# zhibaishouheilab/HealthiVert-GAN

Measured on AMD Instinct MI355X. Metric: sagittal slices/sec (train step, G+D) at 256x256 bs=16, higher is better.
Workload: dtype f16; 1 GPU; two-stage coarse+refine generator + 3x PatchGAN D train step, 256x256, per-GPU bs=16, norm=batch, vanilla GAN; global_batch=16, parallelism=dp1, launch=hipGraph replay (1 graphs/step), 4 streams

## Files before the change

healthivert-gan_amd/csrc/build.py:

```python
import json
import os
import re
import subprocess
import sys
from concurrent.futures import ThreadPoolExecutor

HERE = os.path.dirname(os.path.abspath(__file__))
PKG = os.path.dirname(HERE)
ROOT = os.path.dirname(PKG)
HIPCC = os.environ.get('HIPCC', '/opt/rocm/bin/hipcc')
SOURCES = ['conv_igemm.hip', 'conv_halo.hip', 'conv_halo2.hip', 'conv_lf.hip', 'conv_g4.hip', 'conv_thin.hip', 'conv_px.hip', 'conv_s2t.hip', 'wgrad_halo.hip', 'wgrad_tr.hip', 'conv_narrow.hip', 'conv_head.hip', 'prep.hip', 'norm.hip', 'pointwise.hip', 'attention.hip', 'attention_gram.hip', 'bgemm.hip', 'rhlv.hip', 'assemble.hip', 'infer_prep.hip', 'eval_metrics.hip', 'straighten.hip', 'gen_eval.hip', 'depedicle.hip', 'svm_grade.hip', 'restore.hip', 'spline.hip', 'edt.hip', 'ccl3d.hip', 'morph.hip', 'labelstats.hip', 'filter3d.hip', 'rankfilt.hip', 'resample.hip', 'texture.hip', 'warp.hip', 'similarity.hip', 'shape.hip']
FLAGS = os.environ.get('HV_EXTRA_FLAGS', '').split() + ['--offload-arch=gfx950', '-O3', '-std=c++17', '-fPIC', '-ffp-contract=off', '-Wno-unused-result', '-Wno-inline-asm', '-Rpass-analysis=kernel-resource-usage']
OUT = os.path.join(PKG, 'libhvgan.so')


def _newer(src, dst, deps):
    if not os.path.exists(dst):
        return True
    t = os.path.getmtime(dst)
    return any(os.path.getmtime(p) > t for p in [src] + deps)


def _resources(remarks):
    out, cur = {}, None
    for line in remarks.splitlines():
        m = re.search(r'remark: (?:\S+ )?Function Name: (\S+)', line) or re.search(r'Function Name: (\S+)', line)
        if m:
            cur = out.setdefault(m.group(1), {})
            continue
        if cur is None:
            continue
        for key, pat in (('vgprs', r' VGPRs: (\d+)'), ('agprs', r'AGPRs: (\d+)'), ('scratch', r'ScratchSize \[bytes/lane\]: (\d+)'),
                         ('occupancy', r'Occupancy \[waves/SIMD\]: (\d+)'), ('lds', r'LDS Size \[bytes/block\]: (\d+)')):
            m = re.search(pat, line)
            if m:
                cur[key] = int(m.group(1))
    return out


def build(force=False, verbose=True):
    objdir = os.path.join(HERE, 'build')
    os.makedirs(objdir, exist_ok=True)
    deps = [os.path.join(HERE, 'hv_common.h'), os.path.join(HERE, 'conv_halo.h'), os.path.join(HERE, 'spline_tap.h'), os.path.join(HERE, 'boundary_map.h'), os.path.join(HERE, 'resample_core.h'), os.path.join(ROOT, 'include', 'hvgan.h')]
    jobs = []
    for s in SOURCES:
        src, obj = os.path.join(HERE, s), os.path.join(objdir, s.replace('.hip', '.o'))
        if force or _newer(src, obj, deps):
            jobs.append((src, obj))

    def cc(job):
        src, obj = job
        cmd = [HIPCC] + FLAGS + ['-c', src, '-o', obj]
        if verbose:
            print(' '.join(cmd), flush=True)
        r = subprocess.run(cmd, capture_output=True, text=True)
        if r.returncode != 0:
            raise RuntimeError('hipcc failed for %s:\n%s' % (src, r.stderr[-4000:]))
        with open(obj.replace('.o', '.resources.json'), 'w') as f:
            json.dump(_resources(r.stderr), f, indent=0, sort_keys=True)
        return r.stderr

    with ThreadPoolExecutor(max_workers=4) as ex:
        list(ex.map(cc, jobs))
    objs = [os.path.join(objdir, s.replace('.hip', '.o')) for s in SOURCES]
# ... 13 lines not shown
```

healthivert-gan_amd/csrc/prep.hip:

```cpp
#include <stdlib.h>

#include "hv_common.h"

#define SN_EPS 1e-12f
#define PREP_THREADS 512
#define PREP_MAXK 4608
#define PREP_MAXCO 1024

__device__ __forceinline__ long long wsrc_index(const hv_wprep_layer& L, int co, int ci, int tap) {
    return L.transposed_src ? ((long long)ci * L.Cout + co) * L.taps + tap : ((long long)co * L.Cin + ci) * L.taps + tap;
}

__global__ __launch_bounds__(PREP_THREADS) void weight_prep_kernel(const hv_wprep_layer* __restrict__ layers) {
    const hv_wprep_layer L = layers[blockIdx.x];
    __shared__ float v_s[PREP_MAXK];
    __shared__ float u_s[PREP_MAXCO];
    __shared__ float red[20];
    const int tid = threadIdx.x, lane = tid & 63, wave = tid >> 6, nwave = PREP_THREADS / 64;
    const int K = L.Cin * L.taps;
    float sigma = 1.f;
    if (L.sn) {
        const float* W = L.w_orig;
        for (int i = tid; i < L.Cout; i += PREP_THREADS) u_s[i] = L.u[i];
        for (int i = tid; i < K; i += PREP_THREADS) v_s[i] = L.v[i];
// ... 651 lines not shown
__global__ void fill_kernel(float* p, long long n, float v) {
    long long i = (long long)blockIdx.x * blockDim.x + threadIdx.x;
    const long long st = (long long)gridDim.x * blockDim.x;
    for (; i < n; i += st) p[i] = v;
}
__global__ void axpy_kernel(float* y, const float* x, long long n, float a, int assign) {
    long long i = (long long)blockIdx.x * blockDim.x + threadIdx.x;
    const long long st = (long long)gridDim.x * blockDim.x;
    for (; i < n; i += st) y[i] = assign ? a * x[i] : y[i] + a * x[i];
}
static int ew_grid(long long n) { long long b = (n + 255) / 256; return (int)(b > 4096 ? 4096 : (b < 1 ? 1 : b)); }
extern "C" int hv_fill(float* p, long long n, float value, void* stream) {
    if (!p || n <= 0) return HV_ERR_ARG;
    hipLaunchKernelGGL(fill_kernel, dim3(ew_grid(n)), dim3(256), 0, (hipStream_t)stream, p, n, value);
    HV_LAUNCH_CHECK();
    return HV_OK;
}
extern "C" int hv_axpy(float* y, const float* x, long long n, float a, void* stream) {
    if (!y || !x || n <= 0) return HV_ERR_ARG;
    hipLaunchKernelGGL(axpy_kernel, dim3(ew_grid(n)), dim3(256), 0, (hipStream_t)stream, y, x, n, a, 0);
    HV_LAUNCH_CHECK();
    return HV_OK;
}
__global__ void affine_kernel(float* y, const float* x, long long n, float a, float b) {
    long long i = (long long)blockIdx.x * blockDim.x + threadIdx.x;
    const long long st = (long long)gridDim.x * blockDim.x;
    for (; i < n; i += st) y[i] = a * x[i] + b;
}
extern "C" int hv_affine(float* y, const float* x, long long n, float a, float b, void* stream) {
    if (!y || !x || n <= 0) return HV_ERR_ARG;
    hipLaunchKernelGGL(affine_kernel, dim3(ew_grid(n)), dim3(256), 0, (hipStream_t)stream, y, x, n, a, b);
    HV_LAUNCH_CHECK();
    return HV_OK;
}

__global__ void mul_kernel(float* y, const float* x, const float* z, long long n) {
    long long i = (long long)blockIdx.x * blockDim.x + threadIdx.x;
    const long long st = (long long)gridDim.x * blockDim.x;
    for (; i < n; i += st) y[i] = z ? (y[i] * x[i]) * z[i] : y[i] * x[i];
}
extern "C" int hv_mul(float* y, const float* x, long long n, void* stream) {
    if (!y || !x || n <= 0) return HV_ERR_ARG;
    hipLaunchKernelGGL(mul_kernel, dim3(ew_grid(n)), dim3(256), 0, (hipStream_t)stream, y, x, (const float*)nullptr, n);
    HV_LAUNCH_CHECK();
    return HV_OK;
}
extern "C" int hv_mul3(float* y, const float* x, const float* z, long long n, void* stream) {
    if (!y || !x || !z || n <= 0) return HV_ERR_ARG;
    hipLaunchKernelGGL(mul_kernel, dim3(ew_grid(n)), dim3(256), 0, (hipStream_t)stream, y, x, z, n);
    HV_LAUNCH_CHECK();
    return HV_OK;
}

extern "C" int hv_version(void) { return 106; }
extern "C" const char* hv_arch(void) { return "gfx950"; }
```

healthivert-gan_amd/engine.py:

```python
import contextlib
import ctypes
import os
import types

import torch

from . import lib as _lib
from . import ops
from .lib import ptr, stream
from .ops import Act, rup


def precision_note(precision):
    if precision in ('fp16', 'f16'):
        return 'fp16 MFMA operands / fp32 accumulate; activations and gradients stored as fp16 (image tensors, attention scores, weights, statistics fp32)'
    return 'fp32 MFMA (v_mfma_f32_16x16x4_f32), fp32 storage'


SN_MAX_K, SN_MAX_COUT = 4608, 1024


class ConvParams:

    def __init__(self, name, weight, bias, cin, cout, k, cin_fwd=None, cin_wg=None, u=None, v=None, transposed_src=False):
# ... 300 lines not shown

    def mark(self, a):
        acc = self.accumulates(a)
        self.written.add((id(a.t), a.coff, a.C))
        return acc


class WgradBlock:
    __slots__ = ('side', 'collecting', 'queue', 'later', 'pset')

    def __init__(self):
        self.side, self.collecting, self.queue, self.later, self.pset = None, False, [], [], None

    def open(self, pset, device):
        fork = not SERIAL and torch.cuda.current_stream().cuda_stream not in NO_FORK_STREAMS
        self.side = named_stream('generator-wgrad-block', device) if fork else None
        self.collecting, self.queue, self.later, self.pset = fork, [], [], pset

    def add(self, run):
        self.queue.append(run)

    def before_next_block(self, run):
        if self.collecting:
            self.later.append(run)
        else:
            run()

    def launch(self, keep_collecting=False):
        if self.side is None:
            return
        self.side.wait_stream(torch.cuda.current_stream())
        with torch.cuda.stream(self.side):
            for run in self.queue:
                run()
            self.pset.fold_chain().flush()
        self.queue, self.later, self.collecting = self.later, [], keep_collecting

    def join(self):
        assert not self.queue and not self.later, 'WgradBlock.join(): queued weight gradients were never launched'
        if self.side is not None:
            torch.cuda.current_stream().wait_stream(self.side)
        self.side, self.collecting = None, False


def _wgrad(node, p, xin, gfull, accumulate, prec, dbias=None, dbias_accumulate=False):
    chain = p.owner.fold_chain() if p.owner is not None else None
    if node.transposed:
        ops.conv2d_wgrad(gfull, xin, p.dw, node.k, node.s, node.pad, node.d, accumulate=accumulate, precision=prec, chain=chain)
    else:
        ops.conv2d_wgrad(xin, gfull, p.dw, node.k, node.s, node.pad, node.d, in_shift=node.shift, accumulate=accumulate, precision=prec,
                         dbias=dbias, dbias_accumulate=dbias_accumulate, chain=chain)


def conv_backward(node, book, prec, dbias_accumulate=False, wgrad_accumulate=False, wgrad=True, x_wg=None, premultiplied=False,
                  mul_x=None, dbias_done=False, bn=None):
    p = node.p
    assert bn is None or (node.need_dx and not node.transposed and node.pool_to is None and not node.shift), 'conv_backward: bn= needs the plain data-gradient branch'
    gy = book.twin(node.y)
    want_dbias = p.bias is not None and node.use_bias and wgrad and not dbias_done
    fuse_dbias = want_dbias and not node.transposed and p.coutP == p.cout
    if (node.act != 'none' and not premultiplied) or (want_dbias and not fuse_dbias):
        ops.act_backward(gy, node.y, 'none' if premultiplied else node.act, dbias=p.bias.grad if (want_dbias and not fuse_dbias) else None, dbias_accumulate=dbias_accumulate)
    gfull = Act(gy.t, p.coutP, gy.coff)
    if wgrad:
        xs = node.x if x_wg is None else x_wg
        xin = Act(xs.t, p.cin_wg, xs.coff)
        if book.wgrad_block.collecting:
            book.wgrad_block.add(lambda node=node, p=p, xin=xin, gfull=gfull, acc=wgrad_accumulate, db=p.bias.grad if fuse_dbias else None, dba=dbias_accumulate:
                                 _wgrad(node, p, xin, gfull, acc, prec, dbias=db, dbias_accumulate=dba))
        else:
            _wgrad(node, p, xin, gfull, wgrad_accumulate, prec, dbias=p.bias.grad if fuse_dbias else None, dbias_accumulate=dbias_accumulate)
    if not node.need_dx:
        return
    if node.transposed:
        form = 'src'
    elif node.pool_to is not None and node.pooled(book, prec, 'pool_to'):
        form = 'pool_to'
    elif node.shift:
        form = 'pool' if node.pooled(book, prec, 'pool', mul_x) else 'full'
    else:
        form = 'plain'
    if form == 'full':
        assert not mul_x
        full = node.full_scratch()
        node.dx_call(book, prec, 'full', full, False).launch()
        gx = node.dx_view(book, 'plain')
        ops.copy_channels(full, gx, mode=3, accumulate=book.mark(gx))
    else:
        dst = node.dx_view(book, form)
        node.dx_call(book, prec, form, dst, book.mark(dst), mul_x=mul_x, bn=bn).launch()


_branch_streams = {}


def branch_stream():
    if SERIAL:
        return None
    cur = torch.cuda.current_stream()
    if cur.cuda_stream in NO_FORK_STREAMS:
        return None
    key = cur.device.index
    st = _branch_streams.get(key)
    if st is None:
        st = _branch_streams[key] = named_stream('generator-branch', cur.device)
        NO_FORK_STREAMS.add(st.cuda_stream)
    return st


def chain_link(n, nxt, book, prec):
    if not (nxt is not None and n.need_dx and not n.transposed and nxt.act != 'none'
            and n.x.t is nxt.y.t and n.x.coff == nxt.y.coff and n.p.cin_fwd <= nxt.y.t.shape[-1] - nxt.y.coff):
        return False
    return not n.shift or n.pooled(book, prec, 'pool', nxt.act)


def conv_backward_chain(nodes, book, prec, premultiplied_first=False, stop_before=None):
# ... 168 lines not shown
```

healthivert-gan_amd/models/networks.py:

```python
import functools

import torch
import torch.nn as nn
from torch.nn import init
from torch.optim import lr_scheduler

from ._backend import engine as E
from ._backend import lib as _lib
from ._backend import ops
Act, rup = ops.Act, ops.rup


class Identity(nn.Module):
    def forward(self, x):
        return x


def get_norm_layer(norm_type='instance'):
    if norm_type == 'batch':
        return functools.partial(nn.BatchNorm2d, affine=True, track_running_stats=True)
    if norm_type == 'instance':
        return functools.partial(nn.InstanceNorm2d, affine=False, track_running_stats=False)
    if norm_type == 'none':
        return lambda x: Identity()
# ... 53 lines not shown
    raise NotImplementedError('Generator model name [%s] is not recognized' % netG)


def define_D(input_nc, ndf, netD, n_layers_D=3, norm='batch', init_type='normal', init_gain=0.02, gpu_ids=[]):
    norm_layer = get_norm_layer(norm_type=norm)
    if netD == 'basic':
        net = NLayerDiscriminator(input_nc, ndf, n_layers=3, norm_layer=norm_layer)
    elif netD == 'n_layers':
        net = NLayerDiscriminator(input_nc, ndf, n_layers_D, norm_layer=norm_layer)
    elif netD in ('pixel', 'seg'):
        raise NotImplementedError("define_D('%s'): not on the HealthiVert-GAN hot path" % netD)
    else:
        raise NotImplementedError('Discriminator model name [%s] is not recognized' % netD)
    return init_net(net, init_type, init_gain, gpu_ids)


class _GanLossFn(torch.autograd.Function):
    @staticmethod
    def forward(ctx, pred, target_is_real, mode):
        loss = torch.zeros((), device=pred.device)
        dz = torch.empty_like(pred)
        ops.gan_loss(pred.contiguous(), target_is_real, mode, loss=loss, dz=dz)
        ctx.save_for_backward(dz)
        return loss

    @staticmethod
    def backward(ctx, g):
        (dz,) = ctx.saved_tensors
        return dz * g, None, None


class GANLoss(nn.Module):
    def __init__(self, gan_mode, target_real_label=1.0, target_fake_label=0.0):
        super().__init__()
        self.register_buffer('real_label', torch.tensor(target_real_label))
        self.register_buffer('fake_label', torch.tensor(target_fake_label))
        self.gan_mode = gan_mode
        if gan_mode not in ('lsgan', 'vanilla', 'wgangp'):
            raise NotImplementedError('gan mode %s not implemented' % gan_mode)
        if target_real_label != 1.0 or target_fake_label != 0.0:
            raise NotImplementedError("GANLoss HIP path: labels 1.0 / 0.0")

    def get_target_tensor(self, prediction, target_is_real):
        return (self.real_label if target_is_real else self.fake_label).expand_as(prediction)

    def __call__(self, prediction, target_is_real):
        if self.gan_mode == 'wgangp':
            raise NotImplementedError("GANLoss('wgangp') is not on the HealthiVert-GAN hot path")
        _lib.require_gpu(prediction)
        return _GanLossFn.apply(prediction, bool(target_is_real), self.gan_mode)


CONV_BSTATS = True
HEAD_NORM = True


class _Stem:
    __slots__ = ('p', 'y', 'node')

    def __init__(self, p, y):
        self.p, self.y, self.node = p, y, None


class _Normed:
    __slots__ = ('p', 'node', 'z', 'y', 'stats', 'norm', 'bparts_used', 'head_fused', '_fstats', '_bsums', '_head_ok')

    def __init__(self, p, node, z, y, stats, norm):
        self.p, self.node, self.z, self.y, self.stats, self.norm = p, node, z, y, stats, norm
        self.bparts_used = 0
        self.head_fused = False
        self._fstats = None
        self._bsums = {}
        self._head_ok = {}

    def _partials(self, parts):
        return torch.zeros(max(1, parts) * self.p.cout * 2, dtype=torch.float32, device=self.z.t.device), parts

    def forward_stats(self, prec):
        if self._fstats is None:
            self._fstats = self._partials(int(self.node.stats_parts(prec)))
        return self._fstats if self._fstats[1] else (None, 0)

    def backward_sums(self, consumer, book, prec, mul_x, groups):
        if groups not in self._bsums:
            gx = consumer.dx_view(book, 'plain')
            call = consumer.dx_call(book, prec, 'plain', gx, book.accumulates(gx), mul_x=mul_x, bn=(self.z, self.stats, groups, None))
            self._bsums[groups] = self._partials(call.bstats_parts())
        return self._bsums[groups] if self._bsums[groups][1] else (None, 0)

    def head_call(self, head, prec, groups):
        nm = self.norm
        bn = isinstance(nm, nn.BatchNorm2d)
        xn = (self.stats, nm.weight if bn else None, nm.bias if bn else None, groups if bn else self.z.B, 'lrelu', self.y)
        call = head.node.forward_call(prec, xn=xn, x_raw=self.z)
        if groups not in self._head_ok:
            self._head_ok[groups] = call.supported()
        return call if self._head_ok[groups] else None


class _Logits:
    __slots__ = ('p', 'node', 'y', 'carrier')

    def __init__(self, p, node, y, carrier):
        self.p, self.node, self.y, self.carrier = p, node, y, carrier

    @property
# ... 162 lines not shown
        head = P.layers[-1]
        if head.loss_head_ready:
            want_db = param_grads and head.p.bias is not None and head.node.use_bias
            args = [a for rows, real, loss in ranges for a in (P.logits[rows], real, loss, Act(head.carrier.t[rows], 4, 0))]
            ops.gan_loss_pair(*args, mode=mode, loss_weight=loss_weight, grad_weight=grad_weight, dbias=head.p.bias.grad if want_db else None,
                              dbias_accumulate=accumulate)
            return None, True
        if dz is None:
            dz = torch.empty_like(P.logits)
        for rows, real, loss in ranges:
            ops.gan_loss(P.logits[rows], real, mode, loss=loss, loss_weight=loss_weight, dz=dz[rows], grad_weight=grad_weight)
        return dz, False

    def loss_backward(self, P, target_is_real, mode, loss, grad_weight, need_dx=False, param_grads=True, accumulate=False, loss_weight=1.0, dz=None,
                      backward=True):
        dz, ready = self._loss_seed(P, [(slice(None), target_is_real, loss)], mode, grad_weight, loss_weight, param_grads, accumulate, dz)
        if not backward:
            return None
        return self.run_backward(P, dz, need_dx=need_dx, param_grads=param_grads, accumulate=accumulate, logits_ready=ready)

    def loss_backward_halves(self, P, mode, loss_fake, loss_real, grad_weight, dz=None):
        B = P.B // 2
        dz, ready = self._loss_seed(P, [(slice(0, B), False, loss_fake), (slice(B, None), True, loss_real)], mode, grad_weight, dz=dz)
        return self.run_backward(P, dz, need_dx=False, param_grads=True, accumulate=False, logits_ready=ready)

    def run_backward(self, P, dlogits, need_dx=False, param_grads=True, accumulate=False, logits_ready=False):
        prec = ops.precision_id(self.precision)
        book = P.book
        book.reset()
        B = P.B
        stem, head = P.layers[0], P.layers[-1]
        if not logits_ready:
            ops.copy_channels(Act(dlogits.contiguous().view(B, head.y.H, head.y.W, 1)), head.carrier, mode=0)
        bn = self.norm_kind == 'batch'
        fuse0 = stem.node.act != 'none' and not P.layers[1].node.shift
        sums = (None, 0)
        for li in range(len(P.layers) - 1, 0, -1):
            ent, below = P.layers[li], P.layers[li - 1]
            node = ent.node
            prev_normed = li >= 2 and not node.shift
            if ent is not head:
                nm = ent.norm
                ent.bparts_used = sums[1]
                ops.norm_act_backward(book.twin(ent.y), ent.y, ent.z, book.twin(ent.z), self.norm_kind, P.training, ent.stats,
                                      gamma=nm.weight if bn else None, act='none', dgamma=nm.weight.grad if (bn and param_grads) else None,
                                      dbeta=nm.bias.grad if (bn and param_grads) else None, param_accumulate=accumulate,
                                      groups=P.groups, partials=sums[0], n_partials=sums[1])
            mul_x = stem.node.act if (li == 1 and fuse0) else ('lrelu' if prev_normed else None)
            sums = (None, 0)
            if prev_normed and mul_x and CONV_BSTATS and bn and P.training:
                sums = below.backward_sums(node, book, prec, mul_x, P.groups)
            E.conv_backward(node, book, prec, dbias_accumulate=accumulate, wgrad_accumulate=accumulate, wgrad=param_grads, dbias_done=bool(logits_ready and ent is head),
                            mul_x=mul_x, bn=(below.z, below.stats, P.groups, sums[0]) if sums[1] else None)
        if param_grads:
            ops.copy_channels(P.x_in, P.x4, mode=0)
        stem.node.need_dx = need_dx
        E.conv_backward(stem.node, book, prec, dbias_accumulate=accumulate, wgrad_accumulate=accumulate, wgrad=param_grads,
                        x_wg=P.x4 if param_grads else None, premultiplied=fuse0)
        return book.twin(P.x_in).t.view(B, 1, P.H, P.W) if need_dx else None

    def finish(self):
        for P in self._plans.values():
            P.book.join()
        self.paramset().finish_backward(accumulate=False)
        self.paramset().attach_grads()

    def forward(self, input):
        if torch.is_grad_enabled() and (input.requires_grad or any(p.requires_grad for p in self.parameters())):
            B, _, H, W = input.shape
            P = self.run_forward(input, slot=self._free_plan_slot(B, H, W, input.device))
            anchor = next((p for p in self.parameters() if p.requires_grad), None)
            return _DiscFn.apply(input, anchor, self, P, P.logits)
        return self.run_forward(input).logits.clone()


class _PlanToken:
    """Alive as long as the autograd node that owns a plan's activations is."""


def grads_are_fresh(net):
    ps = list(net.parameters())
    fresh = getattr(ps[0], '_hv_fresh', False) or ps[0].grad is None
    for p in ps:
        p._hv_fresh = False
    return fresh


class _DiscFn(torch.autograd.Function):
    @staticmethod
    def forward(ctx, x, anchor, net, plan, logits):
        import weakref
        ctx.net, ctx.plan, ctx.need_dx = net, plan, x.requires_grad
        ctx.token = _PlanToken()
        plan.pending = weakref.ref(ctx.token)
        return logits.clone()

    @staticmethod
    def backward(ctx, g):
        net, plan = ctx.net, ctx.plan
        if plan.pending is None or plan.pending() is not ctx.token:
            raise RuntimeError("NLayerDiscriminator: the activations of this forward pass were overwritten before its backward ran")
        pg = any(p.requires_grad for p in net.parameters())
        acc = pg and not grads_are_fresh(net)
        S = ops.grad_scale(net.precision)
        pset = net.paramset()
        if acc:
            ops.scale_inplace(pset.flat_grad, S / pset.grad_factor)
        if pg:
            pset.attach_grads()
        dx = net.run_backward(plan, g.contiguous() * S if S != 1.0 else g.contiguous(), need_dx=ctx.need_dx, param_grads=pg, accumulate=acc)
        if pg:
# ... 8 lines not shown
```

healthivert-gan_amd/ops.py:

```python
import ctypes
import os

import torch

from . import lib as _lib
from .lib import ACT, NORM, F16, F32, ptr, stream

_PRECISION = {'fp32': F32, 'f32': F32, 'fp16': F16, 'f16': F16}


_TIMER = None


def timer():
    return _TIMER


def set_timer(t):
    global _TIMER
    _TIMER = t


def default_precision():
    return _PRECISION[os.environ.get('HV_PRECISION', 'fp32').lower()]
# ... 240 lines not shown
            _lib.get().call('hv_wgrad_fold_now', ctypes.byref(f), stream())


FOLD_CHAIN = True


def conv2d_wgrad(x, g, dw, k, stride=1, pad=0, dil=1, in_shift=0, accumulate=False, precision=None, cin=None, cout=None, dbias=None,
                 dbias_accumulate=False, chain=None):
    L = _lib.get()
    d = L.hv_wgrad_desc()
    kh, kw = (k, k) if isinstance(k, int) else k
    d.x = ptr(x.t).value
    d.B, d.H, d.W, d.in_shift = x.B, x.H << in_shift, x.W << in_shift, in_shift
    d.x_ld, d.x_coff, d.Cin = x.ld, x.coff, (x.C if cin is None else cin)
    d.g = ptr(g.t).value
    d.Ho, d.Wo, d.g_ld, d.g_coff, d.Cout = g.H, g.W, g.ld, g.coff, (g.C if cout is None else cout)
    d.KH, d.KW, d.stride, d.pad, d.dil = kh, kw, stride, pad, dil
    d.dw = ptr(dw).value
    d.accumulate = int(accumulate)
    d.precision = precision_id(precision)
    d.dbias = None if dbias is None else ptr(dbias).value
    d.dbias_accumulate = int(dbias_accumulate)
    d.x_f16, d.g_f16 = x.f16, g.f16
    d.workspace, d.workspace_bytes = None, 0
    if chain is not None and not FOLD_CHAIN:
        chain = None
    need = L.size('hv_conv2d_wgrad_workspace_bytes', ctypes.byref(d))
    fold = None
    if chain is not None:
        assert torch.cuda.current_stream(x.t.device).cuda_stream == chain.stream, 'a FoldChain belongs to one stream'
        if chain.pending is not None:
            d.carry = ctypes.pointer(chain.pending)
        if need:
            b, _ = _ws(need, x.t.device, slot=('fold-chain', chain.slot))
            chain.slot ^= 1
            d.workspace, d.workspace_bytes = ptr(b).value, b.numel()
            fold = L.hv_wgrad_fold()
            d.pending = ctypes.pointer(fold)
    elif need:
        b, _ = _ws(need, x.t.device)
        d.workspace, d.workspace_bytes = ptr(b).value, b.numel()
    if _TIMER is not None:
        flops = 2.0 * g.B * g.H * g.W * d.Cout * kh * kw * d.Cin
        nbytes = (2 if x.f16 else 4) * x.B * x.H * x.W * d.Cin + (2 if g.f16 else 4) * g.B * g.H * g.W * d.Cout + 4 * d.Cout * kh * kw * d.Cin
        _TIMER.wrap(('wgrad', x.B, d.H, d.W, d.Cin, d.Cout, kh, stride, dil, 0), flops,
                    lambda: L.call('hv_conv2d_wgrad', ctypes.byref(d), stream()), nbytes)
    else:
        L.call('hv_conv2d_wgrad', ctypes.byref(d), stream())
    if chain is not None:
        chain.pending = fold if (fold is not None and fold.nslabs > 0) else None
    return dw


class LayerTable:

    def __init__(self, struct_name):
        self.struct_name = struct_name
        self.key = None
        self.dev = None
        self.n = 0

    def update(self, rows, key, device):
        if key == self.key:
            return
        L = _lib.get()
        S = getattr(L, self.struct_name)
        arr = (S * len(rows))()
        for i, r in enumerate(rows):
            for f, v in r.items():
                if torch.is_tensor(v):
                    v = ptr(v).value
                setattr(arr[i], f, v)
        raw = bytes(arr)
        host = torch.frombuffer(bytearray(raw), dtype=torch.uint8)
        self.dev = host.to(device)
        self.key, self.n = key, len(rows)

    def ptr(self):
        return ptr(self.dev)


def tiled_elems(rows, taps, K):
    return _lib.get().size('hv_weight_tiled_elems', int(rows), int(taps), int(K))


def tile_weights(w_h, rows, taps, K):
    n = tiled_elems(rows, taps, K)
    if not n:
        return None
    out = torch.empty(n, dtype=torch.float16, device=w_h.device)
    _lib.get().call('hv_weight_tile_f16', ptr(w_h), ptr(out), int(rows), int(taps), int(K), stream())
    return out


def weight_prep(table, max_numel, any_sn=True, any_legacy=True):
    _lib.get().call('hv_weight_prep2', ctypes.cast(table.ptr(), ctypes.POINTER(_lib.get().hv_wprep_layer)), table.n,
                    ctypes.c_longlong(max_numel), int(any_sn), int(any_legacy), stream())


def weight_prep_backward(table, max_numel, any_sn):
    _lib.get().call('hv_weight_prep_backward', ctypes.cast(table.ptr(), ctypes.POINTER(_lib.get().hv_wprep_bwd_layer)), table.n,
                    ctypes.c_longlong(max_numel), int(any_sn), stream())




# ... 160 lines not shown
```

include/hvgan.h:

```cpp
#ifndef HVGAN_H
#define HVGAN_H
#include <stddef.h>
#include <stdint.h>

#ifdef __cplusplus
extern "C" {
#endif

#define HV_OK 0
#define HV_ERR_ARG (-1)
#define HV_ERR_UNSUPPORTED (-2)
#define HV_ERR_WORKSPACE (-3)

enum { HV_F32 = 0, HV_F16 = 1 };
enum { HV_ACT_NONE = 0, HV_ACT_ELU = 1, HV_ACT_RELU = 2, HV_ACT_LRELU = 3, HV_ACT_SIGMOID = 4, HV_ACT_CLAMP = 5 };
enum { HV_NORM_NONE = 0, HV_NORM_BATCH = 1, HV_NORM_INSTANCE = 2 };

int hv_version(void);
const char* hv_arch(void);
int hv_last_kernel_path(void);
const char* hv_last_kernel_name(void);
int hv_set_kernel_timing(void* ev_start, void* ev_stop);
int hv_set_s2t_mode(int mode);

// ... 3 lines not shown
    const float* w; long long w_bstride;
    int Cout, KH, KW, stride, pad, dil, transposed;
    const float* bias;
    const float* ch_scale;
    long long ch_scale_bstride;
    float alpha; int act; int accumulate;
    float* y; int Ho, Wo, y_ld, y_coff;
    int precision;
    const void* w_f16;
    const void* w_f16_tiled;
    const float* mul_src; int mul_ld, mul_coff, mul_act;
    int x_f16, y_f16, mul_f16;
    void* workspace; size_t workspace_bytes;
    float* stats;
    const void* x1;
    int x1_f16, x1_ld, x1_coff;
    const float* w1; int w1_row, w1_tap;
    int pool2;
    const void* bn_x; int bn_x_ld, bn_x_coff;
    const float* bn_stats; int bn_groups;
    float* bstats;
    const float* xn_stats; const float* xn_gamma; const float* xn_beta; int xn_groups, xn_act;
    void* xn_out; int xn_out_ld, xn_out_coff;
} hv_conv_desc;
int hv_conv2d(const hv_conv_desc* d, void* stream);
size_t hv_conv2d_bstats_parts(const hv_conv_desc* d);
size_t hv_conv2d_workspace_bytes(const hv_conv_desc* d);
size_t hv_conv2d_stats_parts(const hv_conv_desc* d);
int hv_last_weight_tables(void);
int hv_conv2d_supported(const hv_conv_desc* d);

typedef struct {
    const float* slabs; float* dw; long long numel; int nslabs; int accumulate;
    const float* bias_slabs; float* dbias; int Cout; int dbias_accumulate;
} hv_wgrad_fold;

typedef struct {
    const float* x; int B, H, W; int in_shift; int x_ld, x_coff, Cin;
    const float* g; int Ho, Wo, g_ld, g_coff, Cout;
    int KH, KW, stride, pad, dil;
    float* dw; int accumulate;
    float* workspace; size_t workspace_bytes;
    int precision;
    int x_f16, g_f16;
    float* dbias; int dbias_accumulate;
    hv_wgrad_fold* pending;
    const hv_wgrad_fold* carry;
} hv_wgrad_desc;
int hv_wgrad_fold_now(const hv_wgrad_fold* fold , void* stream);
size_t hv_conv2d_wgrad_workspace_bytes(const hv_wgrad_desc* d);
int hv_conv2d_wgrad(const hv_wgrad_desc* d, void* stream);

typedef struct {
    const float* w_orig;
    float* u; float* v;
    float* sigma;
    float* w_fwd;
    float* w_bwd;
    void* w_fwd_h; void* w_bwd_h;
    void* w_fwd_t; void* w_bwd_t;
    int Cout, Cin, taps, CinP, CoutF, CoutP, CinB;
    int sn, power_iter, transposed_src;
    void* w_fwd_t2; int K2;
} hv_wprep_layer;
int hv_weight_prep(const hv_wprep_layer* d_layers, int n_layers, long long max_numel, void* stream);
int hv_weight_prep2(const hv_wprep_layer* d_layers, int n_layers, long long max_numel, int any_sn, int any_legacy, void* stream);

size_t hv_weight_tiled_elems(int rows, int taps, int K);
int hv_weight_tile_f16(const void* w_f16, void* w_tiled, int rows, int taps, int K, void* stream);

typedef struct {
    const float* dw_ohwi; const float* w_fwd; const float* u; const float* v; const float* sigma;
    float* dw_orig; int Cout, Cin, taps, CinP, sn, transposed_src, accumulate;
} hv_wprep_bwd_layer;
int hv_weight_prep_backward(const hv_wprep_bwd_layer* d_layers, int n_layers, long long max_numel, int any_sn, void* stream);

size_t hv_head_seed_workspace_bytes(long long npix);
int hv_head_seed_backward(const float* seed, const void* y, int y_f16, int y_ld, int y_coff, void* carrier_f16, long long npix, int act, float* dbias,
                          int dbias_accumulate, float* workspace, size_t workspace_bytes, void* stream);

int hv_act_backward(void* dy, int dy_f16, const void* y, int y_f16 , long long npix, int C, int dy_ld, int dy_coff,
                    int y_ld, int y_coff, int act, float* dbias, int dbias_accumulate, float* workspace, size_t workspace_bytes, void* stream);
size_t hv_act_backward_workspace_bytes(long long npix, int C);

typedef struct {
    const void* x; void* y; int B, HW, C; int x_ld, x_coff, y_ld, y_coff;
    int norm; int training; float eps, momentum;
    const float* gamma; const float* beta; float* running_mean; float* running_var; long long* num_batches_tracked;
    float* stats; int act; int post_sigmoid;
    float* workspace; size_t workspace_bytes;
    int groups;
    int f16;
    const float* partials; int n_partials;
} hv_norm_desc;
size_t hv_norm_workspace_bytes(int B, int HW, int C);
int hv_norm_act_forward(const hv_norm_desc* d, void* stream);
typedef struct {
    const void* dy; const void* y; const void* x; void* dx; int B, HW, C;
    int dy_ld, dy_coff, y_ld, y_coff, x_ld, x_coff, dx_ld, dx_coff;
    int norm; int training; const float* gamma; const float* stats;
    int act; int post_sigmoid;
    float* dgamma; float* dbeta; int param_accumulate;
    float* workspace; size_t workspace_bytes;
    int groups;
    int f16;
    const float* partials; int n_partials;
// ... 393 lines not shown
```

Baseline: 2579 slices/s.

## Add dedicated single-channel stem weight-gradient kernel reading fp32 input directly

Adds a specialized HIP kernel that computes the weight and bias gradient of the Cin=1, 4x4 stride-2 discriminator stem conv. It stages the fp32 input window in LDS and accumulates per-thread partials in fp32, then reduces them through a two-level ticketed cross-workgroup reduction. This removes the channel-padding copy (copy_channels into x4) and the generic padded wgrad path, which waste work on a single input channel. The cost is extra per-block workspace, a ticket buffer, and a finishing step that is serialized through atomics.

```diff
diff --git a/healthivert-gan_amd/csrc/build.py b/healthivert-gan_amd/csrc/build.py
--- a/healthivert-gan_amd/csrc/build.py
+++ b/healthivert-gan_amd/csrc/build.py
@@ -9,7 +9,7 @@
 PKG = os.path.dirname(HERE)
 ROOT = os.path.dirname(PKG)
 HIPCC = os.environ.get('HIPCC', '/opt/rocm/bin/hipcc')
-SOURCES = ['conv_igemm.hip', 'conv_halo.hip', 'conv_halo2.hip', 'conv_lf.hip', 'conv_g4.hip', 'conv_thin.hip', 'conv_px.hip', 'conv_s2t.hip', 'wgrad_halo.hip', 'wgrad_tr.hip', 'conv_narrow.hip', 'conv_head.hip', 'prep.hip', 'norm.hip', 'pointwise.hip', 'attention.hip', 'attention_gram.hip', 'bgemm.hip', 'rhlv.hip', 'assemble.hip', 'infer_prep.hip', 'eval_metrics.hip', 'straighten.hip', 'gen_eval.hip', 'depedicle.hip', 'svm_grade.hip', 'restore.hip', 'spline.hip', 'edt.hip', 'ccl3d.hip', 'morph.hip', 'labelstats.hip', 'filter3d.hip', 'rankfilt.hip', 'resample.hip', 'texture.hip', 'warp.hip', 'similarity.hip', 'shape.hip']
+SOURCES = ['conv_igemm.hip', 'conv_halo.hip', 'conv_halo2.hip', 'conv_lf.hip', 'conv_g4.hip', 'conv_thin.hip', 'conv_px.hip', 'conv_s2t.hip', 'wgrad_halo.hip', 'wgrad_tr.hip', 'wgrad_stem.hip', 'conv_narrow.hip', 'conv_head.hip', 'prep.hip', 'norm.hip', 'pointwise.hip', 'attention.hip', 'attention_gram.hip', 'bgemm.hip', 'rhlv.hip', 'assemble.hip', 'infer_prep.hip', 'eval_metrics.hip', 'straighten.hip', 'gen_eval.hip', 'depedicle.hip', 'svm_grade.hip', 'restore.hip', 'spline.hip', 'edt.hip', 'ccl3d.hip', 'morph.hip', 'labelstats.hip', 'filter3d.hip', 'rankfilt.hip', 'resample.hip', 'texture.hip', 'warp.hip', 'similarity.hip', 'shape.hip']
 FLAGS = os.environ.get('HV_EXTRA_FLAGS', '').split() + ['--offload-arch=gfx950', '-O3', '-std=c++17', '-fPIC', '-ffp-contract=off', '-Wno-unused-result', '-Wno-inline-asm', '-Rpass-analysis=kernel-resource-usage']
 OUT = os.path.join(PKG, 'libhvgan.so')
 
diff --git a/healthivert-gan_amd/csrc/prep.hip b/healthivert-gan_amd/csrc/prep.hip
--- a/healthivert-gan_amd/csrc/prep.hip
+++ b/healthivert-gan_amd/csrc/prep.hip
@@ -727,5 +727,5 @@
     return HV_OK;
 }
 
-extern "C" int hv_version(void) { return 106; }
+extern "C" int hv_version(void) { return 107; }
 extern "C" const char* hv_arch(void) { return "gfx950"; }
diff --git a/healthivert-gan_amd/csrc/wgrad_stem.hip b/healthivert-gan_amd/csrc/wgrad_stem.hip
--- /dev/null
+++ b/healthivert-gan_amd/csrc/wgrad_stem.hip
@@ -0,0 +1,273 @@
+#include "hv_common.h"
+
+typedef float f32x2 __attribute__((ext_vector_type(2)));
+typedef unsigned int stem_u32x4 __attribute__((ext_vector_type(4)));
+
+#define WS_R 4
+#define WS_U 2
+#define WS_GROUP 32
+#define WS_MAX_WG 1024
+#define WS_PART (64 * 16 + 64)
+
+struct WStemK {
+    const float* x; const _Float16* g; float* part; float* gpart; unsigned* tickets; float* dw; float* dbias;
+    int B, H, W, x_ld, x_coff, Ho, Wo, g_ld, g_coff;
+    int rb_per_img, ntiles, nb;
+    int rstep, wstep;
+    int dw_ld, accumulate, dbias_accumulate;
+    unsigned g_bytes;
+};
+
+__device__ __forceinline__ void stem_publish4(float* base, int elem, f32x4 v) {
+    const __amdgpu_buffer_rsrc_t r = __builtin_amdgcn_make_buffer_rsrc(base, 0, WS_PART * 4, 0x00020000);
+    __builtin_amdgcn_raw_buffer_store_b128(__builtin_bit_cast(stem_u32x4, v), r, (unsigned)elem * 4u, 0, 16);
+}
+
+template <int NO>
+__global__ __launch_bounds__(256, 2) void wgrad_stem_kernel(const WStemK p) {
+    constexpr int CO = NO * 8, NDW = CO * 16, PSTEP = 256 / NO;
+    extern __shared__ __attribute__((aligned(16))) float smem[];
+    __shared__ int last;
+    const int tid = threadIdx.x, lane = tid & 63, wave = tid >> 6;
+    const int oct = tid % NO, pix0 = tid / NO;
+    const int WSW = p.W + 2;
+    const int r_init = pix0 / p.Wo, wo_init = pix0 - r_init * p.Wo;
+
+    f32x2 acc[8][8];
+    f32x2 bacc[4];
+#pragma unroll
+    for (int j = 0; j < 8; ++j)
+#pragma unroll
+        for (int t = 0; t < 8; ++t) acc[j][t] = (f32x2){0.f, 0.f};
+#pragma unroll
+    for (int j = 0; j < 4; ++j) bacc[j] = (f32x2){0.f, 0.f};
+
+    const __amdgpu_buffer_rsrc_t gsrc = __builtin_amdgcn_make_buffer_rsrc(const_cast<_Float16*>(p.g), 0, p.g_bytes, 0x00020000);
+    int it_tile = blockIdx.x, it_b = 0, it_base = 0, it_np = 0;
+    auto it_decode = [&]() __attribute__((always_inline)) {
+        it_np = 0;
+        if (it_tile < p.ntiles) {
+            const int n = it_tile / p.rb_per_img, ho0 = (it_tile - n * p.rb_per_img) * WS_R;
+            it_np = min(WS_R, p.Ho - ho0) * p.Wo;
+            it_base = (n * p.Ho + ho0) * p.Wo * p.g_ld + p.g_coff + oct * 8;
+        }
+    };
+    auto issue = [&](stem_u32x4 (&r)[WS_U]) __attribute__((always_inline)) {
+#pragma unroll
+        for (int u = 0; u < WS_U; ++u) {
+            const int pix = pix0 + (it_b * WS_U + u) * PSTEP;
+            r[u] = __builtin_amdgcn_raw_buffer_load_b128(gsrc, pix < it_np ? (unsigned)(it_base + pix * p.g_ld) * 2u : 0x80000000u, 0, 0);
+        }
+        if (++it_b == p.nb) { it_b = 0; it_tile += (int)gridDim.x; it_decode(); }
+    };
+    stem_u32x4 cur[WS_U], nxt[WS_U];
+    it_decode();
+    issue(cur);
+
+    for (int tile = blockIdx.x; tile < p.ntiles; tile += (int)gridDim.x) {
+        const int n = tile / p.rb_per_img, ho0 = (tile - n * p.rb_per_img) * WS_R;
+        const int np = min(WS_R, p.Ho - ho0) * p.Wo;
+        __syncthreads();
+        {
+            const float* xi = p.x + (long long)n * p.H * p.W * p.x_ld + p.x_coff;
+            for (int wc = tid; wc < WSW; wc += 256) {
+                const int wi = wc - 1;
+                const bool cok = (unsigned)wi < (unsigned)p.W;
+#pragma unroll
+                for (int wr = 0; wr < 2 * WS_R + 2; ++wr) {
+                    const int hi = 2 * ho0 - 1 + wr;
+                    float v = 0.f;
+                    if (cok && (unsigned)hi < (unsigned)p.H) v = xi[((long long)hi * p.W + wi) * p.x_ld];
+                    smem[wr * WSW + wc] = (float)(_Float16)v;
+                }
+            }
+        }
+        __syncthreads();
+        int r = r_init, wo = wo_init;
+        auto compute = [&](const stem_u32x4 (&q)[WS_U], int b) __attribute__((always_inline)) {
+#pragma unroll
+            for (int u = 0; u < WS_U; ++u) {
+                const int pix = pix0 + (b * WS_U + u) * PSTEP;
+                const float* wp = smem + (pix < np ? 2 * r * WSW + 2 * wo : 0);
+                f32x2 t[8];
+#pragma unroll
+                for (int kh = 0; kh < 4; ++kh) {
+                    t[2 * kh] = *reinterpret_cast<const f32x2*>(wp + kh * WSW);
+                    t[2 * kh + 1] = *reinterpret_cast<const f32x2*>(wp + kh * WSW + 2);
+                }
+                const f16x8 h = __builtin_bit_cast(f16x8, q[u]);
+                float gf[8];
+#pragma unroll
+                for (int j = 0; j < 8; ++j) gf[j] = (float)h[j];
+#pragma unroll
+                for (int j = 0; j < 4; ++j) bacc[j] += (f32x2){gf[2 * j], gf[2 * j + 1]};
+#pragma unroll
+                for (int j = 0; j < 8; ++j) {
+                    const f32x2 gs = {gf[j], gf[j]};
+#pragma unroll
+                    for (int tp = 0; tp < 8; ++tp) acc[j][tp] = __builtin_elementwise_fma(gs, t[tp], acc[j][tp]);
+                }
+                wo += p.wstep; r += p.rstep;
+                if (wo >= p.Wo) { wo -= p.Wo; ++r; }
+            }
+        };
+        for (int b = 0; b < p.nb; b += 2) {
+            issue(nxt);
+            compute(cur, b);
+            issue(cur);
+            compute(nxt, b + 1);
+        }
+    }
+
+    __syncthreads();
+    float* red = smem;
+#pragma unroll
+    for (int j = 0; j < 8; ++j)
+#pragma unroll
+        for (int tp = 0; tp < 8; ++tp)
+#pragma unroll
+            for (int c = 0; c < 2; ++c) {
+                float v = acc[j][tp][c];
+#pragma unroll
+                for (int o = NO; o < 64; o <<= 1) v += __shfl_xor(v, o, 64);
+                if (lane < NO) red[wave * (NDW + CO) + oct * 128 + j * 16 + tp * 2 + c] = v;
+            }
+#pragma unroll
+    for (int j = 0; j < 8; ++j) {
+        float v = bacc[j >> 1][j & 1];
+#pragma unroll
+        for (int o = NO; o < 64; o <<= 1) v += __shfl_xor(v, o, 64);
+        if (lane < NO) red[wave * (NDW + CO) + NDW + oct * 8 + j] = v;
+    }
+    __syncthreads();
+    const int e4 = tid * 4;
+    const bool has_w = e4 < NDW, has_b = tid < CO;
+    f32x4 s = {0.f, 0.f, 0.f, 0.f};
+    float sb = 0.f;
+#pragma unroll
+    for (int w = 0; w < 4; ++w) {
+        if (has_w) s += *reinterpret_cast<const f32x4*>(red + w * (NDW + CO) + e4);
+        if (has_b) sb += red[w * (NDW + CO) + NDW + tid];
+    }
+    const int bid = blockIdx.x, nwg = gridDim.x;
+    const int grp = bid / WS_GROUP, ngrp = (nwg + WS_GROUP - 1) / WS_GROUP, gsize = min(WS_GROUP, nwg - grp * WS_GROUP);
+    {
+        float* mine = p.part + (long long)bid * WS_PART;
+        if (has_w) stem_publish4(mine, e4, s);
+        if (has_b) hv_publish(mine + NDW + tid, sb);
+    }
+    hv_stores_done();
+    __syncthreads();
+    if (tid == 0) {
+        last = hv_take_ticket_is_last(p.tickets + 1 + grp, (unsigned)gsize);
+        if (last) hv_ticket_reset(p.tickets + 1 + grp);
+    }
+    __syncthreads();
+    if (!last) return;
+    hv_acquire_once();
+    s = (f32x4){0.f, 0.f, 0.f, 0.f};
+    sb = 0.f;
+    for (int k = 0; k < gsize; ++k) {
+        const float* q = p.part + (long long)(grp * WS_GROUP + k) * WS_PART;
+        if (has_w) s += *reinterpret_cast<const f32x4*>(q + e4);
+        if (has_b) sb += q[NDW + tid];
+    }
+    {
+        float* mine = p.gpart + (long long)grp * WS_PART;
+        if (has_w) stem_publish4(mine, e4, s);
+        if (has_b) hv_publish(mine + NDW + tid, sb);
+    }
+    hv_stores_done();
+    __syncthreads();
+    if (tid == 0) {
+        last = hv_take_ticket_is_last(p.tickets, (unsigned)ngrp);
+        if (last) hv_ticket_reset(p.tickets);
+    }
+    __syncthreads();
+    if (!last) return;
+    hv_acquire_once();
+    s = (f32x4){0.f, 0.f, 0.f, 0.f};
+    sb = 0.f;
+    for (int k = 0; k < ngrp; ++k) {
+        const float* q = p.gpart + (long long)k * WS_PART;
+        if (has_w) s += *reinterpret_cast<const f32x4*>(q + e4);
+        if (has_b) sb += q[NDW + tid];
+    }
+    if (has_w) {
+#pragma unroll
+        for (int c = 0; c < 4; ++c) {
+            float* o = p.dw + (long long)(e4 + c) * p.dw_ld;
+            if (p.accumulate) o[0] += s[c];
+            else {
+                o[0] = s[c];
+                for (int q = 1; q < p.dw_ld; ++q) o[q] = 0.f;
+            }
+        }
+    }
+    if (has_b && p.dbias) p.dbias[tid] = p.dbias_accumulate ? p.dbias[tid] + sb : sb;
+}
+
+static int stem_cus() {
+    static int cus = 0;
+    if (!cus) {
+        int dev = 0, n = 0;
+        if (hipGetDevice(&dev) != hipSuccess || hipDeviceGetAttribute(&n, hipDeviceAttributeMultiprocessorCount, dev) != hipSuccess || n <= 0) {
+            (void)hipGetLastError();
+            return 256;
+        }
+        cus = n;
+    }
+    return cus;
+}
+static int stem_tiles(const hv_wgrad_stem_desc* d) { return d->B * hv_cdiv(d->Ho, WS_R); }
+static int stem_workgroups(const hv_wgrad_stem_desc* d) {
+    if (d->workgroups > 0) return d->workgroups;
+    const int t = stem_tiles(d), w = 2 * stem_cus();
+    return t < w ? t : (w < WS_MAX_WG ? w : WS_MAX_WG);
+}
+
+extern "C" int hv_wgrad_stem_eligible(const hv_wgrad_stem_desc* d) {
+    if (!d || !d->x || !d->g || !d->dw) return 0;
+    if (d->precision != HV_F16 || d->x_f16 || !d->g_f16) return 0;
+    if (d->Cin != 1 || d->KH != 4 || d->KW != 4 || d->stride != 2 || d->pad != 1 || d->dil != 1) return 0;
+    if (d->Cout != 32 && d->Cout != 64) return 0;
+    if (d->B <= 0 || d->H <= 0 || d->W <= 0 || (d->H & 1) || (d->W & 1) || d->Ho != d->H / 2 || d->Wo != d->W / 2) return 0;
+    if (d->W > 1024 || d->x_ld < 1 || d->x_coff < 0 || d->x_coff >= d->x_ld || d->dw_ld < 1 || d->dw_ld > 8) return 0;
+    if ((d->g_ld & 7) || (d->g_coff & 7) || d->g_coff < 0 || d->g_coff + d->Cout > d->g_ld || ((uintptr_t)d->g & 15) || ((uintptr_t)d->x & 3) || ((uintptr_t)d->dw & 3)) return 0;
+    if ((long long)d->B * d->Ho * d->Wo * d->g_ld >= (1ll << 30) || (long long)d->B * d->H * d->W * d->x_ld >= (1ll << 40)) return 0;
+    if (d->workgroups < 0 || d->workgroups > WS_MAX_WG) return 0;
+    return 1;
+}
+extern "C" size_t hv_wgrad_stem_workspace_bytes(const hv_wgrad_stem_desc* d) {
+    if (!hv_wgrad_stem_eligible(d)) return 0;
+    const int nwg = stem_workgroups(d);
+    return (size_t)(nwg + hv_cdiv(nwg, WS_GROUP)) * WS_PART * sizeof(float);
+}
+extern "C" int hv_wgrad_stem(const hv_wgrad_stem_desc* d, void* stream) {
+    if (!d || !d->x || !d->g || !d->dw) return HV_ERR_ARG;
+    if (!hv_wgrad_stem_eligible(d)) return HV_ERR_UNSUPPORTED;
+    if (!d->tickets || ((uintptr_t)d->tickets & 3)) return HV_ERR_ARG;
+    const int nwg = stem_workgroups(d);
+    if (!d->workspace || ((uintptr_t)d->workspace & 15) || d->workspace_bytes < hv_wgrad_stem_workspace_bytes(d)) return HV_ERR_WORKSPACE;
+    const int NO = d->Cout / 8, pstep = 256 / NO;
+    WStemK k;
+    k.x = d->x; k.g = reinterpret_cast<const _Float16*>(d->g);
+    k.part = reinterpret_cast<float*>(d->workspace); k.gpart = k.part + (size_t)nwg * WS_PART;
+    k.tickets = reinterpret_cast<unsigned*>(d->tickets); k.dw = d->dw; k.dbias = d->dbias;
+    k.B = d->B; k.H = d->H; k.W = d->W; k.x_ld = d->x_ld; k.x_coff = d->x_coff; k.Ho = d->Ho; k.Wo = d->Wo; k.g_ld = d->g_ld; k.g_coff = d->g_coff;
+    k.rb_per_img = hv_cdiv(d->Ho, WS_R); k.ntiles = stem_tiles(d);
+    k.nb = 2 * hv_cdiv(hv_cdiv((long long)WS_R * d->Wo, pstep), 2 * WS_U);
+    k.rstep = pstep / d->Wo; k.wstep = pstep % d->Wo;
+    k.dw_ld = d->dw_ld; k.accumulate = d->accumulate; k.dbias_accumulate = d->dbias_accumulate;
+    k.g_bytes = (unsigned)((long long)d->B * d->Ho * d->Wo * d->g_ld * 2);
+    const size_t win = (size_t)(2 * WS_R + 2) * (d->W + 2) * sizeof(float), red = (size_t)4 * (NO * 8 * 16 + NO * 8) * sizeof(float);
+    const size_t lds = win > red ? win : red;
+    hv_path_note = 15;
+    HV_KNAME("wgrad_stem_kernel<%d>", NO);
+    HV_TIMING_BEGIN((hipStream_t)stream);
+    if (NO == 8) hipLaunchKernelGGL(wgrad_stem_kernel<8>, dim3(nwg), dim3(256), lds, (hipStream_t)stream, k);
+    else hipLaunchKernelGGL(wgrad_stem_kernel<4>, dim3(nwg), dim3(256), lds, (hipStream_t)stream, k);
+    HV_TIMING_END((hipStream_t)stream);
+    HV_LAUNCH_CHECK();
+    return HV_OK;
+}
diff --git a/healthivert-gan_amd/engine.py b/healthivert-gan_amd/engine.py
--- a/healthivert-gan_amd/engine.py
+++ b/healthivert-gan_amd/engine.py
@@ -376,8 +376,21 @@
                          dbias=dbias, dbias_accumulate=dbias_accumulate, chain=chain)
 
 
+def stem_wgrad_direct(node, book, prec):
+    p = node.p
+    if node.transposed or node.shift or p.cin != 1 or p.coutP != p.cout or p.bias is None or not node.use_bias:
+        return False
+    gy = book.twin(node.y)
+    return ops.wgrad_stem_eligible(node.x, Act(gy.t, p.coutP, gy.coff), p.dw, p.cin_wg, k=node.k, stride=node.s, pad=node.pad, dil=node.d, precision=prec, cin=p.cin)
+
+
+def _wgrad_stem(node, p, gfull, accumulate, prec, dbias, dbias_accumulate):
+    ops.wgrad_stem(node.x, gfull, p.dw, p.cin_wg, chain=p.owner.fold_chain() if p.owner is not None else None, k=node.k, stride=node.s, pad=node.pad,
+                   dil=node.d, accumulate=accumulate, precision=prec, dbias=dbias, dbias_accumulate=dbias_accumulate, cin=p.cin)
+
+
 def conv_backward(node, book, prec, dbias_accumulate=False, wgrad_accumulate=False, wgrad=True, x_wg=None, premultiplied=False,
-                  mul_x=None, dbias_done=False, bn=None):
+                  mul_x=None, dbias_done=False, bn=None, stem_direct=False):
     p = node.p
     assert bn is None or (node.need_dx and not node.transposed and node.pool_to is None and not node.shift), 'conv_backward: bn= needs the plain data-gradient branch'
     gy = book.twin(node.y)
@@ -386,7 +399,14 @@
     if (node.act != 'none' and not premultiplied) or (want_dbias and not fuse_dbias):
         ops.act_backward(gy, node.y, 'none' if premultiplied else node.act, dbias=p.bias.grad if (want_dbias and not fuse_dbias) else None, dbias_accumulate=dbias_accumulate)
     gfull = Act(gy.t, p.coutP, gy.coff)
-    if wgrad:
+    if wgrad and stem_direct:
+        assert x_wg is None and fuse_dbias
+        if book.wgrad_block.collecting:
+            book.wgrad_block.add(lambda node=node, p=p, gfull=gfull, acc=wgrad_accumulate, dba=dbias_accumulate:
+                                 _wgrad_stem(node, p, gfull, acc, prec, p.bias.grad, dba))
+        else:
+            _wgrad_stem(node, p, gfull, wgrad_accumulate, prec, p.bias.grad, dbias_accumulate)
+    elif wgrad:
         xs = node.x if x_wg is None else x_wg
         xin = Act(xs.t, p.cin_wg, xs.coff)
         if book.wgrad_block.collecting:
diff --git a/healthivert-gan_amd/models/networks.py b/healthivert-gan_amd/models/networks.py
--- a/healthivert-gan_amd/models/networks.py
+++ b/healthivert-gan_amd/models/networks.py
@@ -129,6 +129,7 @@
 
 
 CONV_BSTATS = True
+STEM_WGRAD = True
 HEAD_NORM = True
 
 
@@ -397,11 +398,12 @@
                 sums = below.backward_sums(node, book, prec, mul_x, P.groups)
             E.conv_backward(node, book, prec, dbias_accumulate=accumulate, wgrad_accumulate=accumulate, wgrad=param_grads, dbias_done=bool(logits_ready and ent is head),
                             mul_x=mul_x, bn=(below.z, below.stats, P.groups, sums[0]) if sums[1] else None)
-        if param_grads:
+        direct = bool(param_grads and STEM_WGRAD and E.stem_wgrad_direct(stem.node, book, prec))
+        if param_grads and not direct:
             ops.copy_channels(P.x_in, P.x4, mode=0)
         stem.node.need_dx = need_dx
         E.conv_backward(stem.node, book, prec, dbias_accumulate=accumulate, wgrad_accumulate=accumulate, wgrad=param_grads,
-                        x_wg=P.x4 if param_grads else None, premultiplied=fuse0)
+                        x_wg=P.x4 if (param_grads and not direct) else None, premultiplied=fuse0, stem_direct=direct)
         return book.twin(P.x_in).t.view(B, 1, P.H, P.W) if need_dx else None
 
     def finish(self):
diff --git a/healthivert-gan_amd/ops.py b/healthivert-gan_amd/ops.py
--- a/healthivert-gan_amd/ops.py
+++ b/healthivert-gan_amd/ops.py
@@ -316,6 +316,51 @@
     return dw
 
 
+_STEM_TICKETS = {}
+
+
+def _stem_desc(x, g, dw, dw_ld, k=4, stride=2, pad=1, dil=1, accumulate=False, precision=None, dbias=None, dbias_accumulate=False, cin=None, workgroups=0):
+    d = _lib.get().hv_wgrad_stem_desc()
+    kh, kw = (k, k) if isinstance(k, int) else k
+    d.x = ptr(x.t).value
+    d.B, d.H, d.W, d.x_ld, d.x_coff, d.Cin = x.B, x.H, x.W, x.ld, x.coff, (x.C if cin is None else cin)
+    d.g = ptr(g.t).value
+    d.Ho, d.Wo, d.g_ld, d.g_coff, d.Cout = g.H, g.W, g.ld, g.coff, g.C
+    d.KH, d.KW, d.stride, d.pad, d.dil = kh, kw, stride, pad, dil
+    d.dw, d.dw_ld, d.accumulate = ptr(dw).value, dw_ld, int(accumulate)
+    d.dbias = None if dbias is None else ptr(dbias).value
+    d.dbias_accumulate = int(dbias_accumulate)
+    d.precision = precision_id(precision)
+    d.x_f16, d.g_f16 = x.f16, g.f16
+    d.workgroups = workgroups
+    return d
+
+
+def wgrad_stem_eligible(x, g, dw, dw_ld, **kw):
+    return bool(_lib.get().cdll.hv_wgrad_stem_eligible(ctypes.byref(_stem_desc(x, g, dw, dw_ld, **kw))))
+
+
+def wgrad_stem(x, g, dw, dw_ld, chain=None, **kw):
+    L = _lib.get()
+    d = _stem_desc(x, g, dw, dw_ld, **kw)
+    if chain is not None:
+        chain.flush()
+    dev = x.t.device
+    b, _ = _ws(L.size('hv_wgrad_stem_workspace_bytes', ctypes.byref(d)), dev, slot='wgrad-stem')
+    d.workspace, d.workspace_bytes = ptr(b).value, b.numel()
+    key = (str(dev), torch.cuda.current_stream(dev).cuda_stream)
+    t = _STEM_TICKETS.get(key)
+    if t is None:
+        t = _STEM_TICKETS[key] = torch.zeros(64, dtype=torch.int32, device=dev)
+    d.tickets = ptr(t).value
+    if _TIMER is not None:
+        nbytes = 4 * x.B * x.H * x.W + 2 * g.B * g.H * g.W * d.Cout + 4 * d.Cout * 16
+        _TIMER.wrap(('wgrad_stem', x.B, d.H, d.W, 1, d.Cout, 4, 2, 1, 0), 2.0 * g.B * g.H * g.W * d.Cout * 16, lambda: L.call('hv_wgrad_stem', ctypes.byref(d), stream()), nbytes)
+    else:
+        L.call('hv_wgrad_stem', ctypes.byref(d), stream())
+    return dw
+
+
 class LayerTable:
 
     def __init__(self, struct_name):
diff --git a/include/hvgan.h b/include/hvgan.h
--- a/include/hvgan.h
+++ b/include/hvgan.h
@@ -79,6 +79,22 @@
 int hv_conv2d_wgrad(const hv_wgrad_desc* d, void* stream);
 
 typedef struct {
+    const float* x; int B, H, W, x_ld, x_coff, Cin;
+    const void* g; int Ho, Wo, g_ld, g_coff, Cout;
+    int KH, KW, stride, pad, dil;
+    float* dw; int dw_ld; int accumulate;
+    float* dbias; int dbias_accumulate;
+    int precision;
+    int x_f16, g_f16;
+    void* workspace; size_t workspace_bytes;
+    void* tickets;
+    int workgroups;
+} hv_wgrad_stem_desc;
+int hv_wgrad_stem_eligible(const hv_wgrad_stem_desc* d);
+size_t hv_wgrad_stem_workspace_bytes(const hv_wgrad_stem_desc* d);
+int hv_wgrad_stem(const hv_wgrad_stem_desc* d, void* stream);
+
+typedef struct {
     const float* w_orig;
     float* u; float* v;
     float* sigma;
```

Result: no change. 2563 slices/s (-0.6%).
